# jan-frost/uzliti_slam

Hardware: AMD Instinct MI355X
Metric: SE(3) edges optimized/sec (node-pairs matched/sec in `secondary`) (higher is better)
Workload: dtype f64; 1 GPU; BASELINE config 2: 1000-node / 5000-edge SE(3) pose graph, 20 LM iterations, Huber(1) on loop closures; one independent graph per GPU; system_edges=4999

## Files before the change

### uzliti_slam_amd/capi.py

```python
import ctypes as C
import os
import subprocess

import numpy as np

_HERE = os.path.dirname(os.path.abspath(__file__))
LIB_PATH = os.environ.get("UZL_LIB", os.path.join(_HERE, "libuzl_mi355x.so"))
CSRC = os.path.join(_HERE, "csrc")

c_f64p = C.POINTER(C.c_double)
c_i32p = C.POINTER(C.c_int32)
c_u8p = C.POINTER(C.c_uint8)
c_u64p = C.POINTER(C.c_uint64)
c_i64p = C.POINTER(C.c_int64)

UZL_OK = 0
UZL_ERR_BAD_ARG = -1
UZL_ERR_NO_DEVICE = -2
UZL_ERR_HIP = -3
UZL_ERR_NOT_CONVERGED = -4
UZL_ERR_BUSY = -5
UZL_ERR_OOM = -6
UZL_ERR_NOT_FOUND = -7
UZL_ERR_STATE = -8
# ... 538 lines not shown
    def store(self):
        poses = np.empty((self.n, 12)); err = np.empty(max(self.e_in, 1)); used = np.empty(max(self.e_in, 1), np.uint8)
        self._check(self._lib().uzl_pgo_store(self._h, _p(poses, c_f64p), _p(err, c_f64p), _p(used, c_u8p)))
        return poses, err[:self.e_in], used[:self.e_in]

    def get_fixed(self):
        f = np.empty(self.n, np.uint8)
        self._check(self._lib().uzl_pgo_get_fixed(self._h, _p(f, c_u8p)))
        return f

    def set_profiling(self, on):
        self._check(self._lib().uzl_pgo_set_profiling(self._h, C.c_int32(1 if on else 0)))

    def kernel_times(self):
        cap = 64
        names = (C.c_char_p * cap)(); ms = (C.c_double * cap)(); ln = (C.c_int32 * cap)()
        n = self._lib().uzl_pgo_kernel_times(self._h, C.c_int32(cap), names, ms, ln)
        return {names[i].decode(): dict(ms=ms[i], launches=ln[i]) for i in range(max(n, 0))}


class DiagPgo(Pgo):

    _lib = staticmethod(lambda: diag_lib())

    def linearize(self):
        L = self._lib()
        sz = np.zeros(4, np.int32)
        self._check(L.uzl_debug_pgo_linearize(self._h, _p(sz, c_i32p), None, None, None, None, None, None, None, None))
        n, nb, ns, _ = (int(v) for v in sz)
        v2b = np.zeros(max(n, 1), np.int32); rp = np.zeros(nb + 1, np.int32); col = np.zeros(max(ns, 1), np.int32)
        blk = np.zeros((max(ns, 1), 6, 6)); haa = np.zeros((max(nb, 1), 6, 6)); b = np.zeros((max(nb, 1), 6))
        sc = np.zeros(2); P = np.zeros((max(n, 1), 12))
        self._check(L.uzl_debug_pgo_linearize(self._h, _p(sz, c_i32p), _p(v2b, c_i32p), _p(rp, c_i32p), _p(col, c_i32p), _p(blk, c_f64p),
                                              _p(haa, c_f64p), _p(b, c_f64p), _p(sc, c_f64p), _p(P, c_f64p)))
        assert tuple(int(v) for v in sz[:3]) == (n, nb, ns), "the structure changed between the two calls"
        return dict(v2b=v2b[:n], row_ptr=rp, col=col[:ns], blk=blk[:ns], haa=haa[:nb], b=b[:nb], chi2=float(sc[0]), diagmax=float(sc[1]),
                    poses=P[:n])

    def solve(self, lam=-1.0):
        n = self.n
        dx = np.zeros((max(n, 1), 6)); info = np.zeros(8)
        self._check(self._lib().uzl_debug_pgo_solve(self._h, C.c_double(lam), _p(dx, c_f64p), _p(info, c_f64p)))
        return dict(dx=dx[:n], its=int(info[0]), converged=bool(info[1]), guard_trips=int(info[3]), lam=float(info[4]),
                    res_ratio=float(info[5]), rz_end=float(info[6]), rz_stop=float(info[7]))

    def reduced(self, lam=-1.0):
# ... 540 lines not shown
```

### uzliti_slam_amd/csrc/pgo_device.hpp

```cpp
#pragma once
#include <hip/hip_runtime.h>
#include <cstdint>
#include "pgo_types.hpp"

namespace uzl {

#if defined(__gfx90a__) || defined(__gfx942__) || defined(__gfx950__)
#define UZL_PUBLISH_SEQ_ORDER __ATOMIC_RELAXED
__device__ __forceinline__ void publish_wait_own_stores() { asm volatile("s_waitcnt vmcnt(0)" ::: "memory"); }
#else
#define UZL_PUBLISH_SEQ_ORDER __ATOMIC_RELEASE
__device__ __forceinline__ void publish_wait_own_stores() { __threadfence_system(); }
#endif



constexpr int kBlk = 256;

struct Q4 { double w, x, y, z; };
struct V3 { double x, y, z; };
struct M33 { double m[9]; };

__device__ __forceinline__ Q4 qmul(const Q4& a, const Q4& b)
{
// ... 293 lines not shown
#pragma unroll
        for (int c = 0; c < 6; c++) {
            double s = 0.;
#pragma unroll
            for (int k = (r > c ? r : c); k < 6; k++) s += Li[k * 6 + r] * Li[k * 6 + c];
            out[r * 6 + c] = s;
        }
}

constexpr double kProgressSafety = 2., kProgressQMax = 0.95;
constexpr double kProgressQTrust = 0.9;
constexpr double kProgressResidual = 0.2;
__device__ __forceinline__ void progress_decide(PgoDev D, double mt, double mr, double rz)
{
    const double rz_prev = D.scal[11];
    double q = (rz_prev > 0. && rz >= 0.) ? sqrt(rz / rz_prev) : kProgressQMax;
    const bool trusted = q <= kProgressQTrust;
    q = fmin(q, kProgressQMax);
    const double gain = kProgressSafety * q / (1. - q);
    const double et = gain * mt, er = gain * mr;
    D.scal[11] = rz; D.scal[14] = et; D.scal[15] = er;
    if (trusted && et <= D.scal[12] && er <= D.scal[13] && rz >= 0.) D.flags[0] = 1;
}
__device__ __forceinline__ void progress_decide_ml(PgoDev D, double m, double rr, double rz)
{
    const double rz_prev = D.scal[11], m_prev = D.scal[15];
    double q = (rz_prev > 0. && rz >= 0.) ? sqrt(rz / rz_prev) : kProgressQMax;
    if (m_prev > 0.) q = fmax(q, m / m_prev);
    const bool trusted = q <= kProgressQTrust;
    q = fmin(q, kProgressQMax);
    const double est = (kProgressSafety * q / (1. - q)) * m;
    D.scal[11] = rz; D.scal[15] = m;
    if (trusted && est <= 1. && rr <= kProgressResidual * D.scal[14] && rz >= 0.) D.flags[0] = 1;
}
__device__ __forceinline__ double progress_unit(const double* __restrict__ scal, int comp)
{
    const double eps = scal[comp < 3 ? 12 : 13];
    return eps > 0. ? 1. / eps : 1e300;
}

__device__ __forceinline__ const LmSlot& slot_of(const LmSlot* __restrict__ slots) { return slots[blockIdx.z]; }
__device__ __forceinline__ const LmSlot& slot_of(const LmSlot& slot) { return slot; }
__device__ __forceinline__ const LmSlot& slot_of(const HostSlot& hs) { return hs.S; }

}
```

### uzliti_slam_amd/csrc/pgo_handle.hpp

```cpp
#pragma once
#include "uzl_common.hpp"
#include "pgo_types.hpp"
#include "pgo_schur.hpp"
#include "pgo_ml_plan.hpp"
#include "pgo_lm.hpp"

#include <algorithm>
#include <chrono>
#include <cstdlib>
#include <cmath>
#include <functional>
#include <limits>
#include <new>
#include <numeric>

namespace uzl {
void k_prepare_nodes(const uzl_node* nodes, int n, int xy, double* pose, hipStream_t s);
void k_prepare_flat_nodes(const double* poses12, int n, double* pose, hipStream_t s);
void k_prepare_edges(const uzl_edge* edges, const int32_t* src, int e, const double* sensors, int ns, int xy, int odom_params,
                     double* zinv, double* info, hipStream_t s);
void k_prepare_flat_edges(const double* meas12, const double* info36, int e, double* zinv, double* info, hipStream_t s);
int k_chi2(const PgoDev& D, const double* pose, double delta, hipStream_t s);
int k_chi2_trial(const PgoDev& D, const double* pose, double delta, hipStream_t s);
hipError_t k_hessian(const PgoDev& D, const double* pose, double delta, int* g_edges, int* g_rows, hipStream_t s, bool with_chi2 = true, hipEvent_t ev_a = nullptr,
// ... 81 lines not shown
    hipStream_t stream = nullptr;
    int32_t n = 0, e_in = 0, e = 0, nb = 0, nslots = 0;
    std::vector<uint8_t> fixed_in, fixed_eff;
    std::vector<int32_t> ij;
    std::vector<int32_t> src;
    struct InEdge { int32_t from, to; uint8_t odom, valid; double w; };
    std::vector<InEdge> in_edges;
    bool in_ready = false;
    int32_t n_sensors_in = 0;
    std::vector<uint8_t> robust;
    std::vector<double> edge_w;
    bool have_graph = false, structure_ready = false;
    int32_t n_gauge = 0;
    DevBuf<double> pose_a, pose_b, pose_init;
    double* cur = nullptr;
    double* trial = nullptr;
    DevBuf<int32_t> d_v2b, d_ei, d_ej, d_src, d_flags;
    SysBufs sys;
    DevBuf<int32_t> d_slot_edge, d_rb_ptr;
    DevBuf<double> d_srec;
    DevBuf<int4> d_smeta;
    bool srec_stale = true;
    DevBuf<double> d_zinv, d_info;
    DevBuf<double> d_part_a, d_part_b, d_part_c, d_scal, d_err, d_out12, d_stage;
    DevBuf<uint8_t> d_robust;
    DevBuf<uzl_node> d_nodes;
    DevBuf<uzl_edge> d_edges;
    PinBuf<PgoHostScal> h_scal;
    PgoHostScal* d_pub = nullptr;
    uint32_t pub_seq = 0;
    PinBuf<double> h_lambda;
    PgoDev D;
    PgoDev Dp;
    double* pbuf[2] = {nullptr, nullptr};
    struct Reduced {
        bool on = false, strong = false, strong_blocks = false;
        int32_t n_int = 0, n_runs = 0, longest_run = 0, n_sep = 0;
        DevBuf<int32_t> run_ptr, run_rows, slotP, slotN, endL, endR, sep_rows, rsrc, inc_ptr, inc;
        DevBuf<double> elim, runout, runblk;
        SysBufs sys;
        SchurDev S;
    } red;
    int prev_pcg_iters = 0;
    double num_its[2] = {-1., -1.};
    int num_last = -1;
    MlPlan mlp;
    bool ml_mult = false;
// ... 13 lines not shown
    int ml_ix = 0;
    bool ml_pending = false;
    hipStream_t stream2 = nullptr;
    bool streams_borrowed = false;
    hipEvent_t ev_lin = nullptr, ev_setup = nullptr;
    DevBuf<double> d_scal2;
    double lambda_now = 0.;
    DevBuf<uint8_t> ml_arena;
    size_t ml_copy_stride = 0;
    DevBuf<MlDev> d_ml;
    bool no_graph = false;
    int32_t rank = 0, world = 1;
    uzl_allreduce_fn allreduce = nullptr;
    void* allreduce_user = nullptr;
    void* rccl_comm = nullptr;
    bool sharded = false;
    DevBuf<double> d_red;
    int64_t iter_span = 0;
    int64_t l1_span = 0;
    double structure_ms = 0., exchange_ms = 0.;
    int32_t exchange_calls = 0;
    bool structure_reused = false;
    double last_residual_ratio = 0.;
    int32_t guard_trips = 0;
    uint64_t structure_gen = 0;
    bool mult_banned = false;
    KernelTimer timer;
    uzl::LmRun* lm = nullptr;
    LmSlot ml_slot{};
    LmShape ml_shape{};
    uint64_t ml_slot_gen = ~0ull;
    bool last_structure_reused = false;
    std::chrono::steady_clock::time_point t_start;
};

namespace uzl {
inline double pgo_tol_f2(const uzl_pgo_cfg& c) { return c.pcg_stop == 1 ? 1. : kTolFloor2; }
inline double pgo_eps_t(const uzl_pgo_cfg& c) { return c.pcg_stop == 1 ? 0. : kStepT * c.pcg_tol; }
inline double pgo_eps_r(const uzl_pgo_cfg& c) { return c.pcg_stop == 1 ? 0. : kStepR * c.pcg_tol; }
int32_t gauge_fix(uzl_pgo* h);
void build_structure(uzl_pgo* h);
void destroy_pcg_graph(uzl_pgo* h);
bool ml_async_level(const uzl_pgo* h);
double ml_rate_drop(const uzl_pgo* h);
int ml_ns_steps_at(int structure_steps, int lm_iteration);
void prepare_optimize(uzl_pgo* h);
// ... 22 lines not shown
```

### uzliti_slam_amd/csrc/pgo_kernels.hip

```cpp
#include <hip/hip_ext.h>
#include <mutex>

#include "pgo_device.hpp"

namespace uzl {

__global__ __launch_bounds__(kBlk) void prepare_nodes_kernel(const uzl_node* __restrict__ nodes, int n,
                                                             int xy_only, double* __restrict__ pose)
{
    const int v = blockIdx.x * kBlk + threadIdx.x;
    if (v >= n) return;
    Pose P = pose_from_T(nodes[v].pose);
    if (xy_only) P = project_xy(P);
    store_pose(pose, v, P);
}

__global__ __launch_bounds__(kBlk) void prepare_flat_nodes_kernel(const double* __restrict__ poses12, int n,
                                                                  double* __restrict__ pose)
{
    const int v = blockIdx.x * kBlk + threadIdx.x;
    if (v >= n) return;
    store_pose(pose, v, pose_from_T(poses12 + (size_t)v * 12));
}

// ... 602 lines not shown
        __syncthreads();
        if (act) {
            const double* __restrict__ m = D.minv + (size_t)a * 36 + r * 6;
            const int g0 = (int)threadIdx.x - r;
            double zz = 0.;
#pragma unroll
            for (int c = 0; c < 6; c++) zz += m[c] * sv[g0 + c];
            D.z[(size_t)a * 6 + r] = zz;
            acc += rv * zz;
        }
    }
    const double tot = block_sum(acc, s4);
    if (threadIdx.x == 0) {
        D.part_b[blockIdx.x] = tot;
        if (blockIdx.x == 0) {
            D.scal[2] = rz;
            D.flags[1] += 1;
            if (bad) { D.flags[0] = 1; D.flags[2] = 1; }
        }
    }
}

__device__ __forceinline__ void oplus_kernel_body(PgoDev D, const double* __restrict__ pose_in,
                                                     double* __restrict__ pose_out, int blk = blockIdx.x, int nblk = gridDim.x)
{
    __shared__ double s4[4];
    const double lambda = D.scal[3];
    double acc = 0.;
    for (int v = blk * kBlk + threadIdx.x; v < D.n; v += nblk * kBlk) {
        Pose P = load_pose(pose_in, v);
        const int a = D.v2b[v];
        if (a >= 0) {
            const double* __restrict__ dx = D.x + (size_t)a * 6;
            const double* __restrict__ bb = D.b + (size_t)a * 6;
            const double d[6] = {dx[0], dx[1], dx[2], dx[3], dx[4], dx[5]};
#pragma unroll
            for (int i = 0; i < 6; i++) acc += d[i] * (lambda * d[i] + bb[i]);
            P = retract_pose(P, d);
        }
        store_pose(pose_out, v, P);
    }
    const double tot = block_sum(acc, s4);
    if (threadIdx.x == 0) D.part_b[blk] = tot;
}
__global__ __launch_bounds__(kBlk) void oplus_kernel(PgoDev D, const double* __restrict__ pose_in, double* __restrict__ pose_out)
{
    oplus_kernel_body(D, pose_in, pose_out);
}

static inline int grid_for(int items, int per_block, int cap)
{
    int g = (items + per_block - 1) / per_block;
    if (g < 1) g = 1;
    return g > cap ? cap : g;
}

__device__ __forceinline__ void residual_guard_kernel_body(PgoDev D);
__global__ __launch_bounds__(kBlk) void hessian_lm_kernel(const LmSlot* __restrict__ slots, int g_rows_launch)
{
    const LmSlot& S = slots[blockIdx.z];
    const LmDev* lm = S.lm;
    if (lm->phase != kLmLin) return;
    const int b = blockIdx.x;
    if (b < g_rows_launch) { if (b < S.g_asm) hessian_rows_body(S.D, S.pose[lm->cur], lm->delta, b); }
    else if (lm->it == 0 && b - g_rows_launch < S.g_edges) chi2_kernel_body(S.D, S.pose[lm->cur], lm->delta, b - g_rows_launch, S.g_edges);
}
__device__ __forceinline__ bool lm_evaluates(const LmDev* lm) { return lm->phase == kLmSolve && lm->flags[0] != 0 && lm->flags[2] == 0; }
__global__ __launch_bounds__(kBlk) void eval_lm_kernel(const LmSlot* __restrict__ slots, int g_oplus_launch)
{
    const LmSlot& S = slots[blockIdx.z];
    const LmDev* lm = S.lm;
    if (!lm_evaluates(lm)) return;
    const int b = blockIdx.x;
    if (b < g_oplus_launch) { if (b < S.g_oplus) oplus_kernel_body(S.D, S.pose[lm->cur], S.pose[lm->cur ^ 1], b, S.g_oplus); }
    else if (b - g_oplus_launch < S.g_edges) chi2_kernel_body<true>(S.D, S.pose[lm->cur], lm->delta, b - g_oplus_launch, S.g_edges);
}
hipError_t kl_linearize(const LmSlot* sl, int nslots, int g_edges, int g_asm, hipStream_t s)
{
    hipLaunchKernelGGL(hessian_lm_kernel, dim3(g_asm + g_edges, 1, nslots), dim3(kBlk), 0, s, sl, g_asm);
    return hipSuccess;
}
void kl_eval(const LmSlot* sl, int nslots, int g_edges, int g_oplus, hipStream_t s)
{
    hipLaunchKernelGGL(eval_lm_kernel, dim3(g_oplus + g_edges, 1, nslots), dim3(kBlk), 0, s, sl, g_oplus);
}

int g_edges_for(int e) { return grid_for(e, kBlk, kMaxPartials); }

int g_oplus_for(int n) { return grid_for(n, kBlk, kMaxPartials); }


void k_prepare_nodes(const uzl_node* nodes, int n, int xy, double* pose, hipStream_t s)
{
    if (n > 0) hipLaunchKernelGGL(prepare_nodes_kernel, dim3((n + kBlk - 1) / kBlk), dim3(kBlk), 0, s, nodes, n, xy, pose);
}
void k_prepare_flat_nodes(const double* poses12, int n, double* pose, hipStream_t s)
{
// ... 194 lines not shown
```

### uzliti_slam_amd/csrc/pgo_lm_kernels.hip

```cpp
#include "pgo_device.hpp"
#include "pgo_lm.hpp"

namespace uzl {

__device__ __forceinline__ void lm_head_decide(const LmSlot& S, LmDev* lm, int phase, double chi, double dmax, int pass_flags)
{
    const int p = lm->pass + 1;
    lm->pass = p;
    double* __restrict__ scal = S.D.scal;
    int need = 0;
    if (phase == kLmLin) {
        scal[4] = chi; scal[6] = dmax;
        if (lm->it == 0) {
            lm->chi_cur = chi; lm->chi2_initial = chi;
            lm->lambda = 1e-5 * dmax;
            lm->ni = 2.;
        }
        lm->adopted = lm->pending ? 1 : 0;
        lm->ix = lm_pass_ix(phase, lm->ix, lm->pending);
        lm->pending = 0;
        if (lm_refresh(lm->it, lm->iterations, lm->sync_rebuild != 0, lm->last_rel, lm->refresh_rel, lm->rate_ref, lm->rate_last, lm->rate_drop)) {
            lm->st_precond_builds++;
            need |= (lm->it == 0 || lm->sync_rebuild) ? (kNeedNumeric | kNeedTrial) : kNeedRebuild;
        }
// ... 32 lines not shown
    __shared__ LmDev L;
    const LmSlot& S = slots[blockIdx.z];
    LmDev* lm = &L;
    constexpr int kLmWords = (int)(sizeof(LmDev) / 8);
    static_assert(sizeof(LmDev) % 8 == 0 && kLmWords <= kBlk, "LmDev is copied as 8-byte words");
    if ((int)threadIdx.x < kLmWords) reinterpret_cast<unsigned long long*>(&L)[threadIdx.x] = reinterpret_cast<const unsigned long long*>(S.lm)[threadIdx.x];
    __syncthreads();
    const int phase = lm->phase;
    double chi = 0., dmax = 0.;
    if (phase == kLmLin) {
        chi = sum_partials(S.D.part_a, S.g_edges, s4);
        double v = 0.;
        for (int i = threadIdx.x; i < S.g_asm; i += kBlk) v = fmax(v, S.D.part_c[i]);
        dmax = block_max(v, s4);
    }
    if (threadIdx.x == 0) lm_head_decide(S, lm, phase, chi, dmax, pass_flags);
    __syncthreads();
    if ((int)threadIdx.x < kLmWords) reinterpret_cast<unsigned long long*>(S.lm)[threadIdx.x] = reinterpret_cast<const unsigned long long*>(&L)[threadIdx.x];
}

constexpr int kTailBlk = 1024;
__global__ __launch_bounds__(kTailBlk) void lm_tail_kernel(const LmSlot* __restrict__ slots)
{
    __shared__ double s4[4], sr[16], sb[16], sscal[16];
    __shared__ LmDev L;
    const LmSlot& S = slots[blockIdx.z];
    LmDev* lm = &L;
    const int tid = threadIdx.x;
    constexpr int kLmWords = (int)(sizeof(LmDev) / 8);
    static_assert(sizeof(LmDev) % 8 == 0 && kLmWords + 16 <= kTailBlk, "LmDev is copied as 8-byte words");
    if (tid < kLmWords) reinterpret_cast<unsigned long long*>(&L)[tid] = reinterpret_cast<const unsigned long long*>(S.lm)[tid];
    else if (tid < kLmWords + 16) sscal[tid - kLmWords] = S.D.scal[tid - kLmWords];
    __syncthreads();
    const bool solving = lm->phase == kLmSolve;
    const bool done = lm->flags[0] != 0;
    const bool eval = solving && done && lm->flags[2] == 0;
    double chi_t = 0., sc = 0., ratio = 0.;
    if (eval) {
        const PgoDev& P = S.Dp;
        const int n = P.nb * 6;
        double rr = 0., bb = 0.;
        for (int i0 = tid; i0 < n; i0 += 8 * kTailBlk) {
            double rv[8], bv[8];
#pragma unroll
            for (int u = 0; u < 8; u++) { const int i = i0 + u * kTailBlk; rv[u] = i < n ? P.r[i] : 0.; bv[u] = i < n ? P.b[i] : 0.; }
#pragma unroll
            for (int u = 0; u < 8; u++) { rr += rv[u] * rv[u]; bb += bv[u] * bv[u]; }
        }
        for (int o = 32; o; o >>= 1) { rr += __shfl_xor(rr, o); bb += __shfl_xor(bb, o); }
        if ((tid & 63) == 0) { sr[tid >> 6] = rr; sb[tid >> 6] = bb; }
        double va = 0., vb = 0.;
        if (tid < kBlk) {
            for (int i = tid; i < S.g_edges; i += kBlk) va += S.D.part_a[i];
            for (int i = tid; i < S.g_oplus; i += kBlk) vb += S.D.part_b[i];
            va = wave_sum(va);
        }
        __syncthreads();
        if (tid < kBlk && (tid & 63) == 0) s4[tid >> 6] = va;
        __syncthreads();
        chi_t = (s4[0] + s4[1]) + (s4[2] + s4[3]);
        if (tid < kBlk) vb = wave_sum(vb);
        __syncthreads();
        if (tid < kBlk && (tid & 63) == 0) s4[tid >> 6] = vb;
        __syncthreads();
        sc = (s4[0] + s4[1]) + (s4[2] + s4[3]);
        rr = 0.; bb = 0.;
        for (int w = 0; w < 16; w++) { rr += sr[w]; bb += sb[w]; }
        ratio = bb > 0. ? rr / bb : 0.;
    }
    __shared__ uint32_t s_seq;
    if (tid == 0) {
        const uint32_t seq = (uint32_t)(lm->tails + 1);
        lm->tails = (int32_t)seq;
        s_seq = seq;
        double* __restrict__ scal = sscal;
        if (solving && !done) {
            if (lm->flags[1] >= lm->max_it) { lm->phase = kLmAnomaly; lm->anomaly_code = 1; lm->flags[0] = 1; }
// ... 55 lines not shown
```

### uzliti_slam_amd/csrc/pgo_types.hpp

```cpp
#pragma once
#include <cstdint>
#include "../../include/uzl_mi355x.h"

namespace uzl {
constexpr size_t kMlLdsLimit = (size_t)140 * 1024;
__host__ __device__ inline size_t ml_comp4_lds(int n2) { return (size_t)6 * (size_t)n2 * 8 + 64; }


constexpr int kMaxPartials = 8192;
constexpr int kProgressEvery = 2;
constexpr int kRowHdr = 24;

struct PgoDev {
    int32_t n, nb, e, nslots;
    int32_t e_begin, e_end;
    int32_t diag_owner;
    int32_t sibling0;
    double* pose;
    double* pose_trial;
    const int32_t* v2b;
    const int32_t* b2v;
    const int32_t* ei;
    const int32_t* ej;
    const double* zinv;
// ... 113 lines not shown
};

enum LmPhase : int32_t {
    kLmLin = 0,
    kLmSolve = 1,
    kLmRetry = 2,
    kLmNeedSetup = 3,
    kLmDone = 4,
    kLmAnomaly = 5
};
enum LmNeed : int32_t { kNeedNumeric = 1, kNeedTrial = 2, kNeedRebuild = 4 };
enum LmPassFlags : int32_t { kPassSetup = 1 , kPassRebuild = 2  };
struct LmDev {
    int32_t flags[4];
    int32_t phase;
    int32_t cur;
    int32_t ix;
    int32_t pass;
    int32_t init_pass, schur_pass, numeric_pass, trial_pass;
    int32_t build_pass, build_ix, build_cur, need;
    int32_t it, qmax, iterations, max_it;
    int32_t pending, adopted, fresh, pcg_last;
    int32_t sync_rebuild, guarded, tails;
    int32_t st_pcg_iterations, st_lm_trials, st_precond_builds, st_iterations_done, st_terminated_early, anomaly_code, pad0;
    double lambda, ni, chi_cur, last_rel;
    double lambda_setup[2];
    double rate_ref, rate_last;
    double chi2_initial, tol_f2, eps_t, eps_r, refresh_rel, tol2, lambda_retake, delta;
    double scal2[8];
    double rate_drop;
};
struct LmHost {
    LmDev lm;
    double scal[8];
    uint32_t seq_begin, seq;
};
struct LmSlot {
    PgoDev D;
    PgoDev Dp;
    SchurDev SD;
    LmDev* lm;
    LmHost* pub;
    MlHot hot[2];
    const MlDev* dml[2];
    double* rg[2][2];
    double* dense[2][kMlMaxLevels + 1];
    double* nsT[2];
    double* nsX[2];
    double* pbuf[2];
    double* pose[2];
    int32_t g_edges, g_asm, g_oplus, g_rows, g_spmv, red, pad0, pad1;
    int64_t copy_stride;
};
struct HostSlot {
    LmSlot S;
    int32_t ix, cur;
    double tol2;
};

constexpr int32_t kBreakdownIx = 2;
struct PcgArgs {
    int32_t* flags;
    double* scal;
    double* part_a;
    double* part_b;
    double* part_c;
    const int32_t* rowhdr;
    double* hdiag;
    double* z;
    double* blk;
    double* pbuf[2];
    double* r;
    double* x;
    double* xs;
// ... 41 lines not shown
```

### uzliti_slam_amd/csrc/uzl_pgo.hip

```cpp
#include "pgo_handle.hpp"
#include "pgo_lm.hpp"
#include "uzl_streams.hpp"

#include <array>

using namespace uzl;

#include <dlfcn.h>
#include <exception>
#include <system_error>
#include <thread>
namespace {
struct RcclApi {
    typedef struct { char internal[UZL_RCCL_UNIQUE_ID_BYTES]; } UniqueId;
    typedef void* Comm;
    int (*GetUniqueId)(UniqueId*) = nullptr;
    int (*CommInitRank)(Comm*, int, UniqueId, int) = nullptr;
    int (*CommDestroy)(Comm) = nullptr;
    int (*CommCount)(Comm, int*) = nullptr;
    int (*AllReduce)(const void*, void*, size_t, int, int, Comm, hipStream_t) = nullptr;
    const char* (*GetErrorString)(int) = nullptr;
    static constexpr int kDouble = 8, kSum = 0;
    bool ok = false;
    std::string error;
// ... 62 lines not shown
                                : h->allreduce(ptr, count, (void*)h->stream, h->allreduce_user);
    h->exchange_ms += std::chrono::duration<double, std::milli>(std::chrono::steady_clock::now() - t0).count();
    h->exchange_calls++;
    if (rc != 0) throw HipError{hipErrorUnknown, h->rccl_comm ? "ncclAllReduce failed" : "all-reduce callback failed", __FILE__, __LINE__};
}
void shard_allreduce_chi2(uzl_pgo* h)
{
    if (!h->sharded) return;
    h->d_red.reserve(2);
    UZL_HIP(hipMemcpyAsync(h->d_red.p, h->D.scal + 4, sizeof(double), hipMemcpyDeviceToDevice, h->stream));
    shard_allreduce(h, h->d_red.p, 1);
    UZL_HIP(hipMemcpyAsync(h->D.scal + 4, h->d_red.p, sizeof(double), hipMemcpyDeviceToDevice, h->stream));
}

void alloc_problem(uzl_pgo* h, bool keep_poses = false)
{
    const size_t n = std::max(h->n, 1), e = std::max(h->e, 1);
    const bool cur_b = keep_poses && h->cur != nullptr && h->cur == h->pose_b.p;
    h->pose_a.reserve(n * 8, keep_poses, h->stream); h->pose_b.reserve(n * 8, keep_poses, h->stream); h->pose_init.reserve(n * 8);
    h->d_zinv.reserve(e * 7); h->d_info.reserve(e * 36); h->d_robust.reserve(e);
    h->d_ei.reserve(e); h->d_ej.reserve(e);
    h->d_v2b.reserve(n);
    h->d_part_a.reserve(kMaxPartials); h->d_part_b.reserve(kMaxPartials); h->d_part_c.reserve(2 * kMaxPartials);
    h->d_scal.reserve(16); h->d_flags.reserve(4);
    h->h_scal.reserve(1, hipHostMallocMapped | hipHostMallocCoherent); h->h_lambda.reserve(1);
    memset(h->h_scal.p, 0, sizeof(PgoHostScal));
    UZL_HIP(hipHostGetDevicePointer((void**)&h->d_pub, h->h_scal.p, 0));
    h->cur = cur_b ? h->pose_b.p : h->pose_a.p; h->trial = cur_b ? h->pose_a.p : h->pose_b.p;
}

void flatten_edges(uzl_pgo* h)
{
    h->ij.clear(); h->src.clear(); h->robust.clear(); h->edge_w.clear();
    const int n_nodes = h->n, n_edges = (int)h->in_edges.size();
    for (int pass = 0; pass < 2; pass++) {
        for (int k = 0; k < n_edges; k++) {
            const uzl_pgo::InEdge& ed = h->in_edges[k];
            if (ed.from < 0 || ed.to < 0 || ed.from >= n_nodes || ed.to >= n_nodes) continue;
            if (ed.from == ed.to) continue;
            if ((pass == 0) != (ed.odom != 0)) continue;
            if (ed.odom) {
                if (h->fixed_in[ed.from] && !h->fixed_in[ed.to]) continue;
            } else {
                if (!ed.valid) continue;
                if (h->fixed_in[ed.from] && h->fixed_in[ed.to]) continue;
            }
// ... 540 lines not shown
    h->t_start = std::chrono::steady_clock::now();
    h->structure_ms = 0.; h->exchange_ms = 0.; h->exchange_calls = 0;
    h->last_structure_reused = h->structure_ready;
    if (!h->structure_ready) {
        const auto ts = std::chrono::steady_clock::now();
        h->fixed_eff = h->fixed_in;
        h->n_gauge = gauge_fix(h);
        build_structure(h);
        h->structure_ms += std::chrono::duration<double, std::milli>(std::chrono::steady_clock::now() - ts).count();
    }
    if (h->srec_stale) {
        k_slot_records(h->d_zinv.p, h->d_info.p, h->e, h->d_slot_edge.p, h->nslots, h->d_srec.p, h->stream);
        h->srec_stale = false;
    }
}
int do_optimize(uzl_pgo* h, int32_t iterations, uzl_pgo_stats* st)
{
    if (!h->have_graph) return fail(h, UZL_ERR_STATE, "optimize before add_graph/set_graph");
    UZL_HIP(hipSetDevice(h->cfg.device));
    if (iterations <= 0) iterations = h->cfg.iterations;
    prepare_optimize(h);
    uzl_pgo_stats local;
    uzl_pgo_stats* sp = st ? st : &local;
    const int rc = lm_eligible(h) ? do_optimize_lm(h, iterations, sp) : do_optimize_host(h, iterations, sp);
    if (h->red.on && h->red.n_sep >= kSchurStrongMin && sp->lm_trials > 0 && (rc == UZL_OK || rc == UZL_ERR_NOT_CONVERGED)) {
        h->num_last = h->red.strong ? 1 : 0;
        h->num_its[h->num_last] = (h->red.strong_blocks ? 1.3 : 1.) * (double)sp->pcg_iterations / sp->lm_trials;
    }
    return rc;
}
int do_optimize_host(uzl_pgo* h, int32_t iterations, uzl_pgo_stats* st)
{
    const auto t0 = h->t_start;
    uzl_pgo_stats S;
    memset(&S, 0, sizeof(S));
    S.structure_reused = h->last_structure_reused ? 1 : 0;
    S.n_vertices = h->n; S.n_edges = h->e; S.n_gauge_fixed = h->n_gauge;
    hipStream_t s = h->stream;
    PgoDev& D = h->D;
    PgoDev& Dp = h->Dp;
    const bool red = h->red.on;
    const SchurDev& SD = h->red.S;
    S.n_eliminated = red ? h->red.n_int : 0; S.reduced_strong = (red && h->red.strong) ? 1 : 0;
    auto schur_reduce = [&]() { kl_schur_reduce(host_slot(h), h->ml_shape, s, &h->timer); };
    const double delta = h->cfg.huber_delta;
    h->timer.reset();
// ... 909 lines not shown
    const size_t n6 = (size_t)Dp.nb * 6, g6 = (size_t)h->mlp.n[gl] * 6;
    int32_t fl[4] = {0, 0, 0, 0};
    UZL_HIP(hipMemcpyAsync(x, Dp.x, sizeof(double) * n6, hipMemcpyDeviceToHost, s));
    UZL_HIP(hipMemcpyAsync(r, Dp.r, sizeof(double) * n6, hipMemcpyDeviceToHost, s));
    UZL_HIP(hipMemcpyAsync(z, Dp.z, sizeof(double) * n6, hipMemcpyDeviceToHost, s));
    UZL_HIP(hipMemcpyAsync(p, h->pbuf[k & 1], sizeof(double) * n6, hipMemcpyDeviceToHost, s));
    UZL_HIP(hipMemcpyAsync(rg, h->mlb[0].rg[(k & 1) ^ 1], sizeof(double) * g6, hipMemcpyDeviceToHost, s));
    UZL_HIP(hipMemcpyAsync(fl, Dp.flags, sizeof(fl), hipMemcpyDeviceToHost, s));
    UZL_HIP(hipGetLastError());
    UZL_HIP(hipStreamSynchronize(s));
    info[3] = fl[0]; info[4] = fl[1]; info[5] = lam;
    return UZL_OK;
    UZL_GUARD_END(h)
}

extern "C" UZL_DIAG_EXPORT int uzl_debug_pgo_ban_mult(uzl_pgo* h)
{
    UZL_GUARD_BEGIN(h)
    if (h->have_graph) return fail(h, UZL_ERR_STATE, "ban_mult: before the first graph");
    h->mult_banned = true;
    return UZL_OK;
    UZL_GUARD_END(h)
}
#endif

struct uzl_pgo_batch : HandleBase {
    uzl_pgo_cfg cfg;
    std::vector<uzl_pgo*> h;
    hipStream_t stream = nullptr;
    hipStream_t stream2 = nullptr;
    int32_t resident = 0;
    int32_t last_batched = 0;
    uzl::LmRun* lm = nullptr;
    hipStream_t stream_b = nullptr, stream2_b = nullptr;
    uzl::LmRun* lm_b = nullptr;
    KernelTimer timer;
};

static int batch_optimize(uzl_pgo_batch* b, int32_t iterations, uzl_pgo_stats* stats, int32_t* n_batched)
{
    const int B = (int)b->h.size();
    if (n_batched) *n_batched = 0;
    for (uzl_pgo* h : b->h) if (!h->have_graph) return fail(b, UZL_ERR_STATE, "optimize before every graph of the batch has been set");
    UZL_HIP(hipSetDevice(b->cfg.device));
    for (int g = 0; g < B; g++) {
        uzl_pgo* h = b->h[g];
// ... 165 lines not shown
```

### uzliti_slam_amd/csrc/uzl_pgo_lm.hip

```cpp
#include "pgo_handle.hpp"

namespace uzl {

struct LmRun {
    int nslots = 0;
    DevBuf<LmSlot> d_slots;
    DevBuf<LmDev> d_lm;
    PinBuf<LmHost> h_pub;
    LmHost* d_pub = nullptr;
    PinBuf<LmDev> h_init;
    std::vector<LmSlot> slots;
    LmShape shape{};
    DevBuf<double> d_start;
    hipEvent_t ev_fork = nullptr, ev_join = nullptr;
    bool join_pending = false;
    uint64_t gen = ~0ull;
    int solves_of_gen = 0;
    int first_solve_its = 0;
    std::vector<std::vector<int>> trial_its_prev, trial_its_cur;
    std::vector<uint64_t> hist_gen;
    struct Seg { hipGraph_t g = nullptr; hipGraphExec_t x = nullptr; };
    Seg setup, reb, pcg_long[2];
    void drop(Seg& q) { if (q.x) { (void)hipGraphExecDestroy(q.x); q.x = nullptr; } if (q.g) { (void)hipGraphDestroy(q.g); q.g = nullptr; } }
    void drop_all() { drop(setup); drop(reb); drop(pcg_long[0]); drop(pcg_long[1]); }
// ... 80 lines not shown
}

}

LmSlot make_slot(const uzl_pgo* h, LmDev* d_lm, LmHost* d_pub)
{
    LmSlot S;
    memset(&S, 0, sizeof(S));
    S.D = h->D; S.Dp = h->Dp;
    if (d_lm) { S.D.flags = d_lm->flags; S.Dp.flags = d_lm->flags; }
    S.D.pose = nullptr; S.D.pose_trial = nullptr; S.Dp.pose = nullptr; S.Dp.pose_trial = nullptr;
    S.SD = h->red.S; S.red = h->red.on ? 1 : 0;
    S.lm = d_lm; S.pub = d_pub;
    for (int c = 0; c < 2; c++) {
        S.hot[c] = h->mlb[c].hot; S.dml[c] = h->mlb[c].dml;
        S.rg[c][0] = h->mlb[c].rg[0]; S.rg[c][1] = h->mlb[c].rg[1];
        for (int l = 0; l <= kMlMaxLevels; l++) S.dense[c][l] = h->ml_dense_ptr[c][l];
        S.nsT[c] = h->mlb[c].nsT; S.nsX[c] = h->mlb[c].nsX;
    }
    S.pbuf[0] = h->pbuf[0]; S.pbuf[1] = h->pbuf[1];
    S.pose[0] = h->pose_a.p; S.pose[1] = h->pose_b.p;
    S.g_edges = g_edges_for(h->e); S.g_asm = h->D.n_rb; S.g_oplus = g_oplus_for(h->n);
    S.g_rows = g_ml_rows(h->Dp.nb, h->mlp.agg); S.g_spmv = g_ml_spmv(h->Dp.nb, h->mlp.agg);
    S.copy_stride = (int64_t)h->ml_copy_stride;
    return S;
}

LmShape make_shape(const std::vector<uzl_pgo*>& hs, int nslots, bool batch_geometry)
{
    const uzl_pgo* h = hs[0];
    for (const uzl_pgo* g : hs) if (g->mlp.levels >= 1 && g->mlp.n[1] > h->mlp.n[1]) h = g;
    LmShape sh;
    memset(&sh, 0, sizeof(sh));
    sh.nslots = nslots; sh.batch_geometry = batch_geometry ? 1 : 0;
    sh.levels = h->mlp.levels; sh.cl = h->mlp.cl; sh.agg = h->mlp.agg;
    sh.mult = h->ml_mult ? 1 : 0; sh.ns_steps = h->ml_ns_steps; sh.upper_ns = kUpperNs;
    ml_cg_variant(h->mlb[0].hot, h->mlp.agg, h->mlp.lds, &sh.cg_variant, &sh.comp_u, &sh.cg_lds);
    for (const uzl_pgo* g : hs) {
        for (int l = 0; l <= g->mlp.levels; l++) { sh.n_lv[l] = std::max(sh.n_lv[l], g->mlp.n[l]); sh.work_t[l] = std::max(sh.work_t[l], g->mlp.nslots[l] + g->mlp.n[l]); sh.chunks[l] = std::max(sh.chunks[l], g->mlp.chunks[l]); }
        sh.inner_aggs = std::max(sh.inner_aggs, g->mlp.inner_aggs);
        sh.g_edges = std::max(sh.g_edges, g_edges_for(g->e)); sh.g_asm = std::max(sh.g_asm, g->D.n_rb); sh.g_oplus = std::max(sh.g_oplus, g_oplus_for(g->n));
        sh.g_rows = std::max(sh.g_rows, g_ml_rows(g->Dp.nb, g->mlp.agg)); sh.g_spmv = std::max(sh.g_spmv, g_ml_spmv(g->Dp.nb, g->mlp.agg));
        if (g->red.on) {
            const SchurDev& SD = g->red.S;
            sh.red = 1;
            sh.schur_runs = std::max(sh.schur_runs, SD.n_runs);
// ... 143 lines not shown
    bool lin_ahead = false;
    while (n_active > 0) {
        const auto tp0 = std::chrono::steady_clock::now();
        int pf = 0, want = 0;
        bool any_start = false;
        for (int sl = 0; sl < nS; sl++) {
            if (slot_job[sl] < 0 || jobs[slot_job[sl]].finished) continue;
            const LmDev& v = snap[sl].lm;
            int w;
            if (v.phase == kLmSolve) {
                w = solve_passes[sl] == 0 ? kStep : std::min(std::max(kStep, (v.flags[1] / 2 + 1) & ~1), 4 * kLong);
                solve_passes[sl]++;
            } else {
                any_start = true; solve_passes[sl] = 0;
                if (v.phase == kLmNeedSetup) pf |= ((v.need & (kNeedNumeric | kNeedTrial)) ? kPassSetup : 0) | ((v.need & kNeedRebuild) ? kPassRebuild : 0);
                else if (v.phase == kLmLin) {
                    if (lm_refresh(v.it, v.iterations, v.sync_rebuild != 0, v.last_rel, v.refresh_rel, v.rate_ref, v.rate_last, v.rate_drop))
                        pf |= (v.it == 0 || v.sync_rebuild) ? kPassSetup : kPassRebuild;
                    if (v.it > 0 && v.lambda > kLambdaRetake * v.lambda_setup[v.ix ^ (v.pending ? 1 : 0)]) pf |= kPassSetup;
                } else if (v.phase == kLmRetry) {
                    if (v.lambda > kLambdaRetake * v.lambda_setup[v.ix]) pf |= kPassSetup;
                }
                const bool no_history = jobs[(size_t)slot_job[sl]].h->cfg.pass_history == 1;
                auto up = [&](int count) { return nS == 1 ? count + 1 : ((count + 2) & ~1); };
                w = v.pcg_last > 0 ? up(v.pcg_last) : ((R->first_solve_its > 0 && !no_history) ? up(R->first_solve_its) : 2 * kLong);
                if (v.pcg_last > 0 && prev_last[sl] > 0 && v.pcg_last > prev_last[sl]) w = up(v.pcg_last + std::min(v.pcg_last - prev_last[sl], 16));
                {
                    const std::vector<int>& hist = R->trial_its_prev[(size_t)slot_job[sl]];
                    if (!no_history && (size_t)v.st_lm_trials < hist.size()) w = std::max(w, up(hist[(size_t)v.st_lm_trials]));
                }
                w = std::min(w, ((v.max_it + 1) & ~1));
            }
            want = std::max(want, w);
        }
        want = std::max(2, want);
        const int base = (nS == 1 && slot_job[0] >= 0 && snap[0].lm.phase == kLmSolve) ? snap[0].lm.flags[1] : 0;
        static const bool wrong_ix = diag_flag("UZL_LM_WRONG_IX");
        const int pass_ix = lm_pass_ix(snap[0].lm.phase, snap[0].lm.ix, snap[0].lm.pending) ^ (wrong_ix ? 1 : 0);
        const double tol2 = snap[0].lm.tol2;
        mark(0);
        if (any_start && R->join_pending) { UZL_HIP(hipStreamWaitEvent(s, R->ev_join, 0)); R->join_pending = false; }
        mark(1);
        if (any_start) enq_head(R, pf, lin_ahead, s);
        lin_ahead = false;
        mark(2);
        if (pf & kPassSetup) {
            const int steps = nS == 1 ? ml_ns_steps_at(R->shape.ns_steps, snap[0].lm.it) : R->shape.ns_steps;
// ... 68 lines not shown
        double acc[7] = {0, 0, 0, 0, 0, 0, 0};
        static const char* nm[7] = {"wait for the rebuild (0->1)", "linearise + head (1->2)", "set-up / fork (2->3)", "init (3->4)", "pcg (4->5)", "tail (5->6)", "between passes (6->0)"};
        static const bool each = diag_flag("UZL_PHASES_EACH");
        for (size_t i = 0; i + 1 < ph_ev.size(); i++) {
            float ms = 0.f; (void)hipEventElapsedTime(&ms, ph_ev[i], ph_ev[i + 1]); acc[ph_tag[i] % 7] += ms;
            if (each) fprintf(stderr, "%s%d:%.0f", ph_tag[i] == 0 ? "\n[uzl_pgo]   " : " ", ph_tag[i], 1e3 * ms);
        }
        if (each) fprintf(stderr, "\n");
        fprintf(stderr, "[uzl_pgo] segments over %d passes (GPU event time, ms):", passes);
        for (int k = 0; k < 7; k++) fprintf(stderr, "  %s %.3f", nm[k], acc[k]);
        fprintf(stderr, "\n");
        for (hipEvent_t e : ph_ev) (void)hipEventDestroy(e);
    }
    return passes;
}

void finish_job(LmJob& J, uzl_pgo_stats* st, double wall_ms)
{
    uzl_pgo* h = J.h;
    const LmDev& v = J.last.lm;
    h->cur = v.cur ? h->pose_b.p : h->pose_a.p; h->trial = v.cur ? h->pose_a.p : h->pose_b.p;
    h->prev_pcg_iters = v.pcg_last;
    h->last_residual_ratio = J.last.scal[7];
    if (!st) return;
    uzl_pgo_stats S;
    memset(&S, 0, sizeof(S));
    S.structure_reused = h->last_structure_reused ? 1 : 0;
    S.n_vertices = h->n; S.n_edges = h->e; S.n_gauge_fixed = h->n_gauge; S.n_eliminated = h->red.on ? h->red.n_int : 0; S.reduced_strong = (h->red.on && h->red.strong) ? 1 : 0;
    S.iterations_done = v.st_iterations_done; S.lm_trials = v.st_lm_trials; S.pcg_iterations = v.st_pcg_iterations;
    S.terminated_early = v.st_terminated_early; S.precond_builds = v.st_precond_builds;
    S.chi2_initial = v.chi2_initial; S.chi2_final = v.chi_cur; S.lambda_final = v.lambda;
    S.lm_passes = J.passes;
    S.solve_ms = wall_ms;
    S.structure_ms = h->structure_ms;
    *st = S;
}

}

bool lm_eligible(const uzl_pgo* h)
{
    return h->cfg.lm_loop != 1 && h->mlp.levels > 0 && !h->sharded && h->nb > 0 && h->e > 0 && h->Dp.nb > 0 && !h->timer.on &&
           h->stream2 != nullptr;
}

int do_optimize_lm(uzl_pgo* h, int32_t iterations, uzl_pgo_stats* st)
// ... 88 lines not shown
```

Baseline: 18.84 million edges/s.

## Fold final PCG stop test into eval and tail kernels to trim one pass iteration

When a single unreduced slot is still solving and its PCG stop flag is not yet set, the eval and LM tail kernels now recompute the convergence verdict themselves from the partial reductions. If the verdict says done, they proceed with evaluation and commit the stop state. This lets the host schedule one fewer PCG iteration per pass (count instead of count+1), removing one iteration's kernels from each pass. The oplus partial sums move to a separate buffer so they no longer collide with the PCG partials. The cost is a redundant fold in both kernels, plus the risk of the two kernels disagreeing on the verdict.

Result: no change. 18.84 million edges/s, median of 2 (+0.0%).

```diff
diff --git a/uzliti_slam_amd/capi.py b/uzliti_slam_amd/capi.py
--- a/uzliti_slam_amd/capi.py
+++ b/uzliti_slam_amd/capi.py
@@ -584,6 +584,11 @@
 class DiagPgo(Pgo):
 
     _lib = staticmethod(lambda: diag_lib())
+
+    def tail_ends(self):
+        out = C.c_int32(0)
+        self._check(self._lib().uzl_debug_pgo_tail_ends(self._h, C.byref(out)))
+        return int(out.value)
 
     def linearize(self):
         L = self._lib()
diff --git a/uzliti_slam_amd/csrc/pgo_device.hpp b/uzliti_slam_amd/csrc/pgo_device.hpp
--- a/uzliti_slam_amd/csrc/pgo_device.hpp
+++ b/uzliti_slam_amd/csrc/pgo_device.hpp
@@ -339,16 +339,71 @@
     D.scal[11] = rz; D.scal[14] = et; D.scal[15] = er;
     if (trusted && et <= D.scal[12] && er <= D.scal[13] && rz >= 0.) D.flags[0] = 1;
 }
-__device__ __forceinline__ void progress_decide_ml(PgoDev D, double m, double rr, double rz)
-{
-    const double rz_prev = D.scal[11], m_prev = D.scal[15];
+struct PcgLook { double rz_prev, m_prev, bb; };
+__device__ __forceinline__ PcgLook pcg_look_load(const double* scal) { PcgLook L; L.rz_prev = scal[11]; L.m_prev = scal[15]; L.bb = scal[14]; return L; }
+__device__ __forceinline__ bool progress_verdict_ml(const PcgLook& L, double m, double rr, double rz)
+{
+    const double rz_prev = L.rz_prev, m_prev = L.m_prev;
     double q = (rz_prev > 0. && rz >= 0.) ? sqrt(rz / rz_prev) : kProgressQMax;
     if (m_prev > 0.) q = fmax(q, m / m_prev);
     const bool trusted = q <= kProgressQTrust;
     q = fmin(q, kProgressQMax);
     const double est = (kProgressSafety * q / (1. - q)) * m;
+    return trusted && est <= 1. && rr <= kProgressResidual * L.bb && rz >= 0.;
+}
+__device__ __forceinline__ void progress_decide_ml(PgoDev D, double m, double rr, double rz)
+{
+    const bool ends = progress_verdict_ml(pcg_look_load(D.scal), m, rr, rz);
     D.scal[11] = rz; D.scal[15] = m;
-    if (trusted && est <= 1. && rr <= kProgressResidual * D.scal[14] && rz >= 0.) D.flags[0] = 1;
+    if (ends) D.flags[0] = 1;
+}
+
+struct PcgStop {
+    double rz, m;
+    bool look, done, breakdown;
+};
+__device__ __forceinline__ PcgStop pcg_stop_decide(const PcgLook& L, int it, int n_grp, const double* grp_rz, const double* grp_m,
+                                                   const double* grp_rr, double thresh, double rz_last)
+{
+    PcgStop st;
+    st.rz = 0.; st.m = 0.; st.done = false;
+    for (int gi = 0; gi < n_grp; gi++) st.rz += grp_rz[gi];
+    st.look = it % kProgressEvery == 0;
+    if (st.look) {
+        double rr = 0.;
+        for (int gi = 0; gi < n_grp; gi++) { st.m = fmax(st.m, grp_m[gi]); rr += grp_rr[gi]; }
+        st.done = progress_verdict_ml(L, st.m, rr, rz_last);
+    }
+    if (!(st.rz > thresh)) st.done = true;
+    st.breakdown = !(st.rz >= 0.);
+    return st;
+}
+__device__ __forceinline__ void pcg_stop_commit(const PgoDev& D, int it, const PcgStop& st, double rz_last)
+{
+    if (st.look) { D.scal[11] = rz_last; D.scal[15] = st.m; }
+    D.flags[3] = ((it + 1) % kProgressEvery == 0) ? 1 : 0;
+    D.scal[0] = st.rz;
+    if (st.done) D.flags[0] = 1;
+    if (st.breakdown) D.flags[2] = 1;
+}
+__device__ __forceinline__ PcgStop pcg_stop_fold(const PgoDev& D, int n_part, int it, double* sh)
+{
+    constexpr int kGrp = kMaxPartials / 64;
+    const int lane = threadIdx.x & 63, wv = threadIdx.x >> 6, nw = blockDim.x >> 6, n_grp = (n_part + 63) >> 6;
+    const bool look = it % kProgressEvery == 0;
+    const double thresh = D.scal[1], rz_last = D.scal[0];
+    const PcgLook L = pcg_look_load(D.scal);
+    for (int gi = wv; gi < n_grp; gi += nw) {
+        const int i = gi * 64 + lane;
+        const double v = (i < n_part) ? D.part_b[i] : 0.;
+        const double2 x = (look && i < n_part) ? reinterpret_cast<const double2*>(D.part_c)[i] : make_double2(0., 0.);
+        const double s = wave_sum(v), a = wave_max(x.x), b = wave_sum(x.y);
+        if (lane == 0) { sh[gi] = s; sh[kGrp + gi] = a; sh[2 * kGrp + gi] = b; }
+    }
+    __syncthreads();
+    const PcgStop st = pcg_stop_decide(L, it, n_grp, sh, sh + kGrp, sh + 2 * kGrp, thresh, rz_last);
+    __syncthreads();
+    return st;
 }
 __device__ __forceinline__ double progress_unit(const double* __restrict__ scal, int comp)
 {
@@ -359,5 +414,9 @@
 __device__ __forceinline__ const LmSlot& slot_of(const LmSlot* __restrict__ slots) { return slots[blockIdx.z]; }
 __device__ __forceinline__ const LmSlot& slot_of(const LmSlot& slot) { return slot; }
 __device__ __forceinline__ const LmSlot& slot_of(const HostSlot& hs) { return hs.S; }
-
-}
+__device__ __forceinline__ bool lm_stop_pending(const LmSlot& S, const LmDev* lm)
+{
+    return !S.red && lm->phase == kLmSolve && lm->flags[0] == 0 && lm->flags[1] > 0;
+}
+
+}
diff --git a/uzliti_slam_amd/csrc/pgo_handle.hpp b/uzliti_slam_amd/csrc/pgo_handle.hpp
--- a/uzliti_slam_amd/csrc/pgo_handle.hpp
+++ b/uzliti_slam_amd/csrc/pgo_handle.hpp
@@ -127,7 +127,7 @@
     DevBuf<int4> d_smeta;
     bool srec_stale = true;
     DevBuf<double> d_zinv, d_info;
-    DevBuf<double> d_part_a, d_part_b, d_part_c, d_scal, d_err, d_out12, d_stage;
+    DevBuf<double> d_part_a, d_part_b, d_part_c, d_part_s, d_scal, d_err, d_out12, d_stage;
     DevBuf<uint8_t> d_robust;
     DevBuf<uzl_node> d_nodes;
     DevBuf<uzl_edge> d_edges;
@@ -187,6 +187,7 @@
     int32_t exchange_calls = 0;
     bool structure_reused = false;
     double last_residual_ratio = 0.;
+    int32_t last_tail_ends = 0;
     int32_t guard_trips = 0;
     uint64_t structure_gen = 0;
     bool mult_banned = false;
diff --git a/uzliti_slam_amd/csrc/pgo_kernels.hip b/uzliti_slam_amd/csrc/pgo_kernels.hip
--- a/uzliti_slam_amd/csrc/pgo_kernels.hip
+++ b/uzliti_slam_amd/csrc/pgo_kernels.hip
@@ -648,8 +648,10 @@
 }
 
 __device__ __forceinline__ void oplus_kernel_body(PgoDev D, const double* __restrict__ pose_in,
-                                                     double* __restrict__ pose_out, int blk = blockIdx.x, int nblk = gridDim.x)
-{
+                                                     double* __restrict__ pose_out, int blk = blockIdx.x, int nblk = gridDim.x,
+                                                     double* __restrict__ part = nullptr)
+{
+    if (!part) part = D.part_b;
     __shared__ double s4[4];
     const double lambda = D.scal[3];
     double acc = 0.;
@@ -667,7 +669,7 @@
         store_pose(pose_out, v, P);
     }
     const double tot = block_sum(acc, s4);
-    if (threadIdx.x == 0) D.part_b[blk] = tot;
+    if (threadIdx.x == 0) part[blk] = tot;
 }
 __global__ __launch_bounds__(kBlk) void oplus_kernel(PgoDev D, const double* __restrict__ pose_in, double* __restrict__ pose_out)
 {
@@ -694,11 +696,16 @@
 __device__ __forceinline__ bool lm_evaluates(const LmDev* lm) { return lm->phase == kLmSolve && lm->flags[0] != 0 && lm->flags[2] == 0; }
 __global__ __launch_bounds__(kBlk) void eval_lm_kernel(const LmSlot* __restrict__ slots, int g_oplus_launch)
 {
+    __shared__ double sstop[3 * (kMaxPartials / 64)];
     const LmSlot& S = slots[blockIdx.z];
     const LmDev* lm = S.lm;
-    if (!lm_evaluates(lm)) return;
+    if (!lm_evaluates(lm)) {
+        if (!lm_stop_pending(S, lm)) return;
+        const PcgStop st = pcg_stop_fold(S.Dp, S.g_rows, lm->flags[1], sstop);
+        if (!st.done || st.breakdown) return;
+    }
     const int b = blockIdx.x;
-    if (b < g_oplus_launch) { if (b < S.g_oplus) oplus_kernel_body(S.D, S.pose[lm->cur], S.pose[lm->cur ^ 1], b, S.g_oplus); }
+    if (b < g_oplus_launch) { if (b < S.g_oplus) oplus_kernel_body(S.D, S.pose[lm->cur], S.pose[lm->cur ^ 1], b, S.g_oplus, S.part_s); }
     else if (b - g_oplus_launch < S.g_edges) chi2_kernel_body<true>(S.D, S.pose[lm->cur], lm->delta, b - g_oplus_launch, S.g_edges);
 }
 hipError_t kl_linearize(const LmSlot* sl, int nslots, int g_edges, int g_asm, hipStream_t s)
diff --git a/uzliti_slam_amd/csrc/pgo_lm_kernels.hip b/uzliti_slam_amd/csrc/pgo_lm_kernels.hip
--- a/uzliti_slam_amd/csrc/pgo_lm_kernels.hip
+++ b/uzliti_slam_amd/csrc/pgo_lm_kernels.hip
@@ -78,7 +78,7 @@
 constexpr int kTailBlk = 1024;
 __global__ __launch_bounds__(kTailBlk) void lm_tail_kernel(const LmSlot* __restrict__ slots)
 {
-    __shared__ double s4[4], sr[16], sb[16], sscal[16];
+    __shared__ double s4[4], sr[16], sb[16], sscal[16], sstop[3 * (kMaxPartials / 64)];
     __shared__ LmDev L;
     const LmSlot& S = slots[blockIdx.z];
     LmDev* lm = &L;
@@ -89,6 +89,19 @@
     else if (tid < kLmWords + 16) sscal[tid - kLmWords] = S.D.scal[tid - kLmWords];
     __syncthreads();
     const bool solving = lm->phase == kLmSolve;
+    if (lm_stop_pending(S, lm)) {
+        const int it = lm->flags[1];
+        const double rz_last = sscal[0];
+        const PcgStop st = pcg_stop_fold(S.Dp, S.g_rows, it, sstop);
+        if (st.done && tid == 0) {
+            PgoDev V = S.Dp;
+            pcg_stop_commit(V, it, st, rz_last);
+            V.scal = sscal; V.flags = lm->flags;
+            pcg_stop_commit(V, it, st, rz_last);
+            lm->st_tail_ends++;
+        }
+        __syncthreads();
+    }
     const bool done = lm->flags[0] != 0;
     const bool eval = solving && done && lm->flags[2] == 0;
     double chi_t = 0., sc = 0., ratio = 0.;
@@ -108,7 +121,7 @@
         double va = 0., vb = 0.;
         if (tid < kBlk) {
             for (int i = tid; i < S.g_edges; i += kBlk) va += S.D.part_a[i];
-            for (int i = tid; i < S.g_oplus; i += kBlk) vb += S.D.part_b[i];
+            for (int i = tid; i < S.g_oplus; i += kBlk) vb += S.part_s[i];
             va = wave_sum(va);
         }
         __syncthreads();
diff --git a/uzliti_slam_amd/csrc/pgo_types.hpp b/uzliti_slam_amd/csrc/pgo_types.hpp
--- a/uzliti_slam_amd/csrc/pgo_types.hpp
+++ b/uzliti_slam_amd/csrc/pgo_types.hpp
@@ -159,7 +159,8 @@
     int32_t it, qmax, iterations, max_it;
     int32_t pending, adopted, fresh, pcg_last;
     int32_t sync_rebuild, guarded, tails;
-    int32_t st_pcg_iterations, st_lm_trials, st_precond_builds, st_iterations_done, st_terminated_early, anomaly_code, pad0;
+    int32_t st_pcg_iterations, st_lm_trials, st_precond_builds, st_iterations_done, st_terminated_early, anomaly_code;
+    int32_t st_tail_ends;
     double lambda, ni, chi_cur, last_rel;
     double lambda_setup[2];
     double rate_ref, rate_last;
@@ -186,7 +187,8 @@
     double* nsX[2];
     double* pbuf[2];
     double* pose[2];
-    int32_t g_edges, g_asm, g_oplus, g_rows, g_spmv, red, pad0, pad1;
+    int32_t g_edges, g_asm, g_oplus, g_rows, g_spmv, red;
+    double* part_s;
     int64_t copy_stride;
 };
 struct HostSlot {
diff --git a/uzliti_slam_amd/csrc/uzl_pgo.hip b/uzliti_slam_amd/csrc/uzl_pgo.hip
--- a/uzliti_slam_amd/csrc/uzl_pgo.hip
+++ b/uzliti_slam_amd/csrc/uzl_pgo.hip
@@ -108,6 +108,7 @@
     h->d_ei.reserve(e); h->d_ej.reserve(e);
     h->d_v2b.reserve(n);
     h->d_part_a.reserve(kMaxPartials); h->d_part_b.reserve(kMaxPartials); h->d_part_c.reserve(2 * kMaxPartials);
+    h->d_part_s.reserve(kMaxPartials);
     h->d_scal.reserve(16); h->d_flags.reserve(4);
     h->h_scal.reserve(1, hipHostMallocMapped | hipHostMallocCoherent); h->h_lambda.reserve(1);
     memset(h->h_scal.p, 0, sizeof(PgoHostScal));
@@ -694,6 +695,7 @@
     prepare_optimize(h);
     uzl_pgo_stats local;
     uzl_pgo_stats* sp = st ? st : &local;
+    h->last_tail_ends = 0;
     const int rc = lm_eligible(h) ? do_optimize_lm(h, iterations, sp) : do_optimize_host(h, iterations, sp);
     if (h->red.on && h->red.n_sep >= kSchurStrongMin && sp->lm_trials > 0 && (rc == UZL_OK || rc == UZL_ERR_NOT_CONVERGED)) {
         h->num_last = h->red.strong ? 1 : 0;
@@ -1649,6 +1651,15 @@
     return UZL_OK;
     UZL_GUARD_END(h)
 }
+
+extern "C" UZL_DIAG_EXPORT int uzl_debug_pgo_tail_ends(uzl_pgo* h, int32_t* out)
+{
+    UZL_GUARD_BEGIN(h)
+    if (!out) return fail(h, UZL_ERR_BAD_ARG, "tail_ends: null output");
+    *out = h->last_tail_ends;
+    return UZL_OK;
+    UZL_GUARD_END(h)
+}
 #endif
 
 struct uzl_pgo_batch : HandleBase {
diff --git a/uzliti_slam_amd/csrc/uzl_pgo_lm.hip b/uzliti_slam_amd/csrc/uzl_pgo_lm.hip
--- a/uzliti_slam_amd/csrc/uzl_pgo_lm.hip
+++ b/uzliti_slam_amd/csrc/uzl_pgo_lm.hip
@@ -126,6 +126,7 @@
     S.pose[0] = h->pose_a.p; S.pose[1] = h->pose_b.p;
     S.g_edges = g_edges_for(h->e); S.g_asm = h->D.n_rb; S.g_oplus = g_oplus_for(h->n);
     S.g_rows = g_ml_rows(h->Dp.nb, h->mlp.agg); S.g_spmv = g_ml_spmv(h->Dp.nb, h->mlp.agg);
+    S.part_s = h->d_part_s.p;
     S.copy_stride = (int64_t)h->ml_copy_stride;
     return S;
 }
@@ -315,7 +316,8 @@
                     if (v.lambda > kLambdaRetake * v.lambda_setup[v.ix]) pf |= kPassSetup;
                 }
                 const bool no_history = jobs[(size_t)slot_job[sl]].h->cfg.pass_history == 1;
-                auto up = [&](int count) { return nS == 1 ? count + 1 : ((count + 2) & ~1); };
+                static const int pass_extra = diag_int("UZL_LM_PASS_EXTRA", 0);
+                auto up = [&](int count) { return nS == 1 ? count + (sh.red ? 1 : 0) + pass_extra : ((count + 2) & ~1); };
                 w = v.pcg_last > 0 ? up(v.pcg_last) : ((R->first_solve_its > 0 && !no_history) ? up(R->first_solve_its) : 2 * kLong);
                 if (v.pcg_last > 0 && prev_last[sl] > 0 && v.pcg_last > prev_last[sl]) w = up(v.pcg_last + std::min(v.pcg_last - prev_last[sl], 16));
                 {
@@ -430,6 +432,7 @@
     h->cur = v.cur ? h->pose_b.p : h->pose_a.p; h->trial = v.cur ? h->pose_a.p : h->pose_b.p;
     h->prev_pcg_iters = v.pcg_last;
     h->last_residual_ratio = J.last.scal[7];
+    h->last_tail_ends = v.st_tail_ends;
     if (!st) return;
     uzl_pgo_stats S;
     memset(&S, 0, sizeof(S));
```
